# ska-telescope/ska-sdp-func-python

Measured on AMD Instinct MI355X. Metric: Mvis/s gridded (invert, 8k^2 w-stack grid) at 1/2/4/8 MI355X, higher is better.
Workload: dtype f32; 1 GPU; C2: SKA-MID 197 dishes, 64 chan x 100 times per GPU, 4096^2 image, 8192^2 w-stack grid; nvis_per_gpu=123558400, nchan_total=64, npix=4096, support=8, nplanes=9, parallelism=channel-sharded x1, 1 all-reduce

## Files before the change

### include/ska_sdp_hip.h

```cpp
#ifndef SKA_SDP_HIP_H
#define SKA_SDP_HIP_H

#include <stddef.h>
#include <stdint.h>

#ifdef __cplusplus
extern "C" {
#endif

#define SDP_HIP_OK 0
#define SDP_HIP_ERR_INVALID_ARG 1
#define SDP_HIP_ERR_RUNTIME 2
#define SDP_HIP_ERR_NO_DEVICE 3
#define SDP_HIP_ERR_MEMORY 4

#define SDP_HIP_F32 1
#define SDP_HIP_F64 2
#define SDP_HIP_C64 3
#define SDP_HIP_C128 4

#define SDP_HIP_FLIP_UW 1u
#define SDP_HIP_ACCUMULATE 2u
#define SDP_HIP_BATCH_FIRST 4u
#define SDP_HIP_BATCH_LAST 8u
#define SDP_HIP_KEEP_BUCKETS 16u
#define SDP_HIP_REUSE_BUCKETS 32u
#define SDP_HIP_FP32 64u
#define SDP_HIP_W_SLAB 128u
#define SDP_HIP_SLOT1 256u

typedef struct sdp_hip_wgrid_info {
    int support;
    double beta;
    int ngrid_x, ngrid_y;
    int nplanes;
    double w0, dw;
    int64_t nvis_used;
    int64_t nitems;
    int plane_chunk;
    float ms_prep, ms_grid, ms_fft, ms_screen;
    int bucket;
    int grid_launches;
    int padded;
    int fp64;
    int tiled;
    int folded;
    int layout_reused;
} sdp_hip_wgrid_info;

int sdp_hip_version(void);
int sdp_hip_device_count(int *count, char *errbuf, size_t errbuf_len);
int sdp_hip_release_workspace(char *errbuf, size_t errbuf_len);
int sdp_hip_set_stage_timing(int enable);

int sdp_hip_ms2dirty(const double *uvw, int64_t uvw_row_stride,
                     const double *freq, int nchan, int64_t nrow,
                     const void *vis, int vis_dtype, int64_t vis_row_stride,
                     int64_t vis_chan_stride, const void *wgt, int wgt_dtype,
                     int64_t wgt_row_stride, int64_t wgt_chan_stride,
                     int npix_x, int npix_y, double pixsize_x,
                     double pixsize_y, double epsilon, int do_wstacking,
                     unsigned flags, double *dirty, int64_t dirty_stride_x,
                     int64_t dirty_stride_y, void *stream,
                     sdp_hip_wgrid_info *info, char *errbuf,
                     size_t errbuf_len);

int sdp_hip_ms2dirty_batch(const double *uvw, int64_t uvw_row_stride,
                           const double *freq, int nchan, int64_t nrow,
                           const void *vis, int vis_dtype,
                           int64_t vis_row_stride, int64_t vis_chan_stride,
                           const void *wgt, int wgt_dtype, int64_t wgt_row_stride,
                           int64_t wgt_chan_stride, int npix_x, int npix_y,
                           double pixsize_x, double pixsize_y, double epsilon,
                           int do_wstacking, unsigned flags,
                           const double *bounds, double *dirty,
                           int64_t dirty_stride_x, int64_t dirty_stride_y,
                           void *stream, sdp_hip_wgrid_info *info,
                           char *errbuf, size_t errbuf_len);

int sdp_hip_wstack_layout(const double *bounds, int npix_x, int npix_y,
                          double pixsize_x, double pixsize_y, double epsilon,
                          int do_wstacking, unsigned flags, sdp_hip_wgrid_info *info,
                          char *errbuf, size_t errbuf_len);

int sdp_hip_wstack_fingerprint(const double *uvw, int64_t uvw_row_stride, int64_t nrow,
                               const double *freq, int nchan, uint64_t *out,
                               char *errbuf, size_t errbuf_len);

int sdp_hip_ms2dirty_vis(const double *uvw, int64_t uvw_row_stride,
                         const double *freq, int nchan, int64_t nrow,
                         const void *vis, int vis_dtype, int64_t vis_row_stride,
                         int64_t vis_chan_stride, int64_t vis_pol_stride,
                         int npol_vis, const double *pol_coeff, const void *wgt,
                         int wgt_dtype, int64_t wgt_row_stride,
                         int64_t wgt_chan_stride, const void *vis_flags,
                         int flag_bytes, int64_t flag_row_stride,
                         int64_t flag_chan_stride, int64_t flag_pol_stride,
                         int pol, int npix_x, int npix_y, double pixsize_x,
                         double pixsize_y, double epsilon, int do_wstacking,
                         unsigned flags, double *dirty, int64_t dirty_stride_x,
                         int64_t dirty_stride_y, double *sumwt,
                         const double *shift_lmn, void *stream,
                         sdp_hip_wgrid_info *info, char *errbuf,
                         size_t errbuf_len);

int sdp_hip_ms2dirty_vis_batch(const double *uvw, int64_t uvw_row_stride,
                               const double *freq, int nchan, int64_t nrow,
                               const void *vis, int vis_dtype, int64_t vis_row_stride,
                               int64_t vis_chan_stride, int64_t vis_pol_stride,
                               int npol_vis, const double *pol_coeff, const void *wgt,
                               int wgt_dtype, int64_t wgt_row_stride,
                               int64_t wgt_chan_stride, const void *vis_flags,
                               int flag_bytes, int64_t flag_row_stride,
                               int64_t flag_chan_stride, int64_t flag_pol_stride,
                               int pol, int npix_x, int npix_y, double pixsize_x,
                               double pixsize_y, double epsilon, int do_wstacking,
                               unsigned flags, const double *bounds, double *dirty,
                               int64_t dirty_stride_x, int64_t dirty_stride_y,
                               double *sumwt, const double *shift_lmn, void *stream,
                               sdp_hip_wgrid_info *info, char *errbuf,
                               size_t errbuf_len);

int sdp_hip_ms2dirty_vis_pols(const double *uvw, int64_t uvw_row_stride,
                              const double *freq, int nchan, int64_t nrow,
                              const void *vis, int vis_dtype, int64_t vis_row_stride,
                              int64_t vis_chan_stride, int64_t vis_pol_stride,
                              int npol_vis, const double *pol_coeff, int npol_img,
                              const void *wgt, int wgt_dtype, int64_t wgt_row_stride,
                              int64_t wgt_chan_stride, int64_t wgt_pol_stride,
                              const void *vis_flags, int flag_bytes,
// ... 294 lines not shown
```

### ska-sdp-func-python_amd/csrc/wstack.hip

```cpp
#include <hipcub/hipcub.hpp>
#include <hipfft/hipfft.h>

#include <algorithm>
#include <cmath>
#include <cstdio>
#include <cstdlib>
#include <functional>
#include <memory>
#include <mutex>
#include <tuple>
#include <type_traits>
#include <vector>

#include "sdp_common.h"
#include "wstack_fx_fft.h"
#include "wstack_types.h"
#include "wstack_bucket.h"

namespace sdp {
namespace wstack {

__global__ __launch_bounds__(64) void k_sum_slots(const double *__restrict__ slots, double *out) {
    double s = 0.0;
    for (int i = threadIdx.x; i < kSumSlots; i += 64) s += slots[i];
// ... 1065 lines not shown
                const float2 h = fbuf[fx_pad(X < 0 ? X + g.ngx : X)];
                if (g.do_w) {
                    const double l = X * g.px, r2 = l * l + m2;
                    const double sp = r2 < 1.0 ? r2 / (sqrt(1.0 - r2) + 1.0) - g.s0 : 0.0;
                    double ph = wq * sp;
                    ph -= rint(ph);
                    double sn, cs;
                    sincospi_t<float2>(2.0 * ph, &sn, &cs);
                    acc[m] += (double)h.x * cs - (double)h.y * sn;
                } else {
                    acc[m] += (double)h.x;
                }
            }
        }
        __syncthreads();
    }
#pragma unroll
    for (int m = 0; m < PX; ++m) {
        const int ix = t + m * S::T;
        if (ix < g.nx) {
            const PixelGeom p = pixel_geom(g, ix, iy, tab);
            const double res = p.inside ? acc[m] * p.corr : 0.0;
            double *o = dirty + ix * sx + iy * sy;
            *o = accumulate ? *o + res : res;
        }
    }
}

template <int LOGN>
__global__ __launch_bounds__(FxShape<LOGN>::T) __attribute__((amdgpu_waves_per_eu(4, 8))) void
k_screen_adj_xfft(Geo g, const double *__restrict__ dirty, int64_t sx, int64_t sy, int p_begin,
                  int np, float2 *__restrict__ spec, const double *__restrict__ tab,
                  const float2 *__restrict__ twg) {
    using S = FxShape<LOGN>;
    extern __shared__ float2 fbuf[];
    const int t = threadIdx.x, iy = blockIdx.x;
    float2 *const twl = fx_twl<LOGN>(fbuf, twg, t);
    float val[8];
#pragma unroll
    for (int e = 0; e < 8; ++e) {
        const int r = e < 4 ? e : e + 8;
        const int i = t + r * S::T;
        const int X = i < g.ngx / 2 ? i : i - g.ngx, ix = X + g.nx / 2;
        val[e] = 0.0f;
        if (ix >= 0 && ix < g.nx) {
            const PixelGeom p = pixel_geom(g, ix, iy, tab);
            val[e] = p.inside ? (float)(dirty[ix * sx + iy * sy] * p.corr) : 0.0f;
        }
    }
    const double mm = (iy - g.ny / 2) * g.py, m2 = mm * mm;
    const int64_t tplane = (int64_t)g.ny * g.ngx;
    const int pt = fx_pad(t);
    for (int q = 0; q < np; ++q) {
        const double wq = g.w0 + (p_begin + q) * g.dw;
        int tt = t;
        asm volatile("" : "+v"(tt));
        float2 v[16];
#pragma unroll
        for (int r = 0; r < 16; ++r) v[r] = make_float2(0.0f, 0.0f);
#pragma unroll
        for (int e = 0; e < 8; ++e) {
            const int r = e < 4 ? e : e + 8;
            const int i = tt + r * S::T;
            const int X = i < g.ngx / 2 ? i : i - g.ngx;
            if (val[e] != 0.0f) {
                if (g.do_w) {
                    const double l = X * g.px, r2 = l * l + m2;
                    const double sp = r2 / (sqrt(1.0 - r2) + 1.0) - g.s0;
                    double ph = wq * sp;
                    ph -= rint(ph);
                    double sn, cs;
                    sincospi_t<float2>(2.0 * ph, &sn, &cs);
                    v[r] = make_float2((float)(val[e] * cs), (float)(-val[e] * sn));
                } else {
                    v[r] = make_float2(val[e], 0.0f);
                }
            }
        }
        fx_fft<LOGN, -1>(v, fbuf, twl, t);
        float2 *o = spec + q * tplane + (int64_t)iy * g.ngx;
#pragma unroll
        for (int r = 0; r < 16; ++r) o[t + r * S::T] = fbuf[fx_padc<S::T>(t, pt, r * S::T)];
        __syncthreads();
    }
}

__device__ __forceinline__ void store_vis(float2 *p, float2 v, int accumulate) {
    if (accumulate) {
        const float2 o = *p;
        v.x += o.x;
        v.y += o.y;
    }
    *p = v;
}
__device__ __forceinline__ void store_vis(double2 *p, float2 v, int accumulate) {
    double2 w = make_double2(v.x, v.y);
    if (accumulate) {
        const double2 o = *p;
        w.x += o.x;
        w.y += o.y;
    }
    *p = w;
}
__device__ __forceinline__ void store_vis_d(float2 *p, double xr, double xi, int accumulate) {
    float2 w = make_float2((float)xr, (float)xi);
    if (accumulate) {
        const float2 o = *p;
        w.x += o.x;
        w.y += o.y;
    }
    *p = w;
}
__device__ __forceinline__ void store_vis_d(double2 *p, double xr, double xi, int accumulate) {
    double2 w = make_double2(xr, xi);
    if (accumulate) {
        const double2 o = *p;
        w.x += o.x;
        w.y += o.y;
    }
    *p = w;
}

struct OutConv {
    int npv = 1;
    int64_t vps = 0;
    double cre[4] = {1.0, 0.0, 0.0, 0.0}, cim[4] = {0.0, 0.0, 0.0, 0.0};
};

template <class VT>
__global__ void k_zero_vis(int64_t nrow, int nchan, VT *vis, int64_t vrs, int64_t vcs,
                           OutConv oc) {
    const int64_t v = blockIdx.x * (int64_t)blockDim.x + threadIdx.x;
    if (v >= nrow * nchan) return;
    const int64_t row = v / nchan;
    const int chan = (int)(v - row * nchan);
    VT z;
    z.x = 0;
    z.y = 0;
    for (int k = 0; k < oc.npv; ++k) vis[row * vrs + chan * vcs + k * oc.vps] = z;
}

template <class VT>
__global__ void k_finalize(int64_t n, int nchan,
                           const VisRec *__restrict__ recs, const float2 *__restrict__ acc, VT *vis,
                           int64_t vrs, int64_t vcs, int accumulate, OutConv oc) {
    for (int64_t r = blockIdx.x * (int64_t)blockDim.x + threadIdx.x; r < n;
         r += (int64_t)gridDim.x * blockDim.x) {
        const VisRec rc = recs[r];
        const float2 a = acc[r];
        const float2 v = make_float2(rc.cre * a.x - rc.cim * a.y, rc.cre * a.y + rc.cim * a.x);
        const int64_t row = rc.idx / (uint32_t)nchan;
        const int chan = (int)(rc.idx - row * nchan);
        VT *p = vis + row * vrs + chan * vcs;
        if (oc.npv == 1 && oc.cre[0] == 1.0 && oc.cim[0] == 0.0) {
            store_vis(p, v, accumulate);
            continue;
        }
        for (int k = 0; k < oc.npv; ++k) {
            if (oc.cre[k] == 0.0 && oc.cim[k] == 0.0) continue;
            const double xr = oc.cre[k] * v.x - oc.cim[k] * v.y;
            const double xi = oc.cre[k] * v.y + oc.cim[k] * v.x;
            store_vis_d(p + k * oc.vps, xr, xi, accumulate);
        }
    }
}

// ... 2632 lines not shown
    });
}

static void degrid_f64(const Plan &P, int p_lo, int p_hi, void *vis, int vis_dtype, int64_t vrs,
                int64_t vcs, int accumulate, const OutConv &oc, hipStream_t st) {
    SDP_REQUIRE(P.mfma64, "the fp64 predict needs one-cell buckets");
    dispatch_int<kMinW64, kMaxW64>(P.g.W, [&](auto w) {
        constexpr int W = decltype(w)::value;
        auto go = [&](auto *v) {
            using VT = std::remove_pointer_t<decltype(v)>;
            if (P.g.do_w)
                launch_degrid_f64_mfma<W, true, VT>(P, p_lo, p_hi, v, vrs, vcs, accumulate, oc, st);
            else
                launch_degrid_f64_mfma<W, false, VT>(P, p_lo, p_hi, v, vrs, vcs, accumulate, oc, st);
        };
        if (vis_dtype == SDP_HIP_C128) go(static_cast<double2 *>(vis));
        else go(static_cast<float2 *>(vis));
    });
}

static float2 *degrid_sink() {
    static float2 *sinks[64] = {};
    int dev = 0;
    SDP_HIP_CHECK(hipGetDevice(&dev));
    SDP_REQUIRE(dev >= 0 && dev < 64, "device index out of range");
    static std::mutex mu;
    std::lock_guard<std::mutex> lock(mu);
    if (!sinks[dev])
        SDP_HIP_CHECK(hipMalloc(&sinks[dev], (size_t)kDegridSinkBlocks * 64 * sizeof(float2)));
    return sinks[dev];
}

template <int W, bool WS>
static void launch_degrid_mfma(const Plan &P, int p_lo, int p_hi, float2 *acc, hipStream_t st) {
    const size_t lds = degrid_lds_bytes<W, WS>();
    const auto r = chunk_items(P, p_lo, p_hi);
    const unsigned per = P.subsort ? 16u : 1u;
    const unsigned n = per * (r.second - r.first);
    if (n == 0) return;
    float2 *const sink = degrid_sink();
    if (P.vdirect)
        k_degrid_mfma<W, WS, true><<<n, 64, lds, st>>>(
            P.g, P.recs, n, P.pt.fitems + per * (size_t)r.first, P.grid, p_lo, p_hi, P.vdirect, sink);
    else
        k_degrid_mfma<W, WS, false><<<n, 64, lds, st>>>(
            P.g, P.recs, n, P.pt.fitems + per * (size_t)r.first, P.grid, p_lo, p_hi, acc, sink);
}

static void grid_f32(const Plan &P, int p_lo, int p_hi, hipStream_t st) {
    dispatch_int<2, kMaxW>(P.g.W, [&](auto w) {
        constexpr int W = decltype(w)::value;
        if (P.g.do_w) launch_grid_mfma_pad<W, true>(P, p_lo, p_hi, st);
        else launch_grid_mfma_pad<W, false>(P, p_lo, p_hi, st);
    });
}

static void degrid_f32(const Plan &P, int p_lo, int p_hi, float2 *acc, hipStream_t st) {
    dispatch_int<2, kMaxW>(P.g.W, [&](auto w) {
        constexpr int W = decltype(w)::value;
        if (P.g.do_w) launch_degrid_mfma<W, true>(P, p_lo, p_hi, acc, st);
        else launch_degrid_mfma<W, false>(P, p_lo, p_hi, acc, st);
    });
}

static void fill_info(const Plan &P, sdp_hip_wgrid_info *info) {
    if (!info) return;
    info->support = P.g.W;
    info->beta = P.g.beta;
    info->ngrid_x = P.g.ngx;
    info->ngrid_y = P.g.ngy;
    info->nplanes = P.g.nplanes;
    info->w0 = P.g.w0;
    info->dw = P.g.dw;
    info->nvis_used = P.pt.nrec;
    info->nitems = P.pt.nitems;
    info->plane_chunk = P.chunk_planes;
    info->bucket = P.g.sub;
    info->padded = (P.pad4 || P.subpad || P.pad64) ? 1 : 0;
    info->fp64 = P.f64 ? 1 : 0;
    info->tiled = P.g.tiled;
    info->grid_launches = (P.g.nplanes + P.chunk_planes - 1) / P.chunk_planes;
    info->folded = P.g.fold;
    info->layout_reused = 0;
}

static void exec_fft(hipfftHandle h, bool f64, void *in, void *out, int direction) {
    const hipfftResult r =
        f64 ? hipfftExecZ2Z(h, (hipfftDoubleComplex *)in, (hipfftDoubleComplex *)out, direction)
            : hipfftExecC2C(h, (hipfftComplex *)in, (hipfftComplex *)out, direction);
    if (r != HIPFFT_SUCCESS) throw Error(SDP_HIP_ERR_RUNTIME, "hipfftExec failed");
}

static void *plane_ptr(const Plan &P, int q, size_t e) {
    return reinterpret_cast<char *>(P.grid) +
           ((size_t)q * P.g.ngx * P.g.ngy + e) * cbytes(P);
}

static void fft_rows_y(const Plan &P, int q0, int np, int direction, hipStream_t st) {
    const Geo &g = P.g;
    const int nrow = P.row_hi - P.row_lo;
    if (nrow <= 0) return;
    hipfftHandle hr = fft_plan_1d(g.ngy, 1, g.ngy, nrow, st, P.f64);
    for (int q = q0; q < q0 + np; ++q) {
        void *p = plane_ptr(P, q, (size_t)P.row_lo * g.ngy);
        exec_fft(hr, P.f64, p, p, direction);
    }
}

static void fft_rows_x(const Plan &P, int np, int direction, hipStream_t st,
                       void *in = nullptr) {
    const Geo &g = P.g;
    hipfftHandle hc = fft_plan_1d(g.ngx, 1, g.ngx, np * g.ny, st, P.f64);
    exec_fft(hc, P.f64, in ? in : (void *)P.spec, P.spec, direction);
}

static void zero_band(const Plan &P, int np, hipStream_t st) {
    const Geo &g = P.g;
    if (P.row_hi <= P.row_lo || np <= 0) return;
    const size_t width = (size_t)(P.row_hi - P.row_lo) * g.ngy * cbytes(P);
    for (int q = 0; q < np; ++q)
        SDP_HIP_CHECK(hipMemsetAsync(plane_ptr(P, q, (size_t)P.row_lo * g.ngy), 0, width, st));
    if (P.core.p)
        SDP_HIP_CHECK(hipMemsetAsync(P.core.p, 0,
                                     (size_t)np * P.core.nx * P.core.ny * sizeof(double2), st));
}

static void setup_core(Plan &P) {
    P.core = CoreAcc{nullptr, 0, 0, 0, 0};
    const int cw = env_int("SDP_HIP_CORE", 128);
    if (P.f64 || cw <= 0) return;
    const Geo &g = P.g;
    const int x0 = std::max(P.row_lo, g.ngx / 2 - cw / 2), x1 = std::min(P.row_hi, g.ngx / 2 + cw / 2);
    const int y0 = std::max(0, g.ngy / 2 - cw / 2), y1 = std::min(g.ngy, g.ngy / 2 + cw / 2);
    if (x1 <= x0 || y1 <= y0) return;
    P.core = CoreAcc{scratch<double>("core64", (size_t)P.chunk_planes * (x1 - x0) * (y1 - y0) * 2),
                     x0, x1 - x0, y0, y1 - y0};
}

__global__ __launch_bounds__(256) void k_core_merge(float2 *__restrict__ grid, int ngx, int ngy,
                                                    CoreAcc c, int q0, int np) {
    const int64_t per = (int64_t)c.nx * c.ny, n = per * np;
    for (int64_t i = blockIdx.x * (int64_t)blockDim.x + threadIdx.x; i < n;
         i += (int64_t)gridDim.x * blockDim.x) {
        const int q = (int)(i / per);
        const int64_t e = i - q * per;
        const int x = (int)(e / c.ny), y = (int)(e - (int64_t)x * c.ny);
        const double2 v = reinterpret_cast<const double2 *>(c.p)[(int64_t)(q0 + q) * per + e];
        float2 &o = grid[((int64_t)(q0 + q) * ngx + c.x0 + x) * ngy + c.y0 + y];
        o = make_float2((float)((double)o.x + v.x), (float)((double)o.y + v.y));
    }
}

static void core_merge(const Plan &P, int q0, int np, hipStream_t st) {
    if (!P.core.p || np <= 0) return;
    const int64_t n = (int64_t)P.core.nx * P.core.ny * np;
    k_core_merge<<<(unsigned)std::min<int64_t>((n + 255) / 256, 8192), 256, 0, st>>>(
        P.grid, P.g.ngx, P.g.ngy, P.core, q0, np);
    SDP_HIP_CHECK(hipGetLastError());
}

static dim3 tr_grid(const Geo &g, int xrows, int np) {
    return dim3((unsigned)((xrows + kTr - 1) / kTr), (unsigned)((g.ny + kTr - 1) / kTr),
                (unsigned)np);
}

static bool tr16(const Geo &g) {
// ... 30 lines not shown
        k_tr_t_to_grid<double2><<<grd, blk, 0, st>>>(
            g, reinterpret_cast<const double2 *>(P.spec),
            static_cast<double2 *>(plane_ptr(P, q0, 0)), P.row_lo, P.row_hi);
    else if (tr16(g))
        k_tr_t_to_grid16<<<tr_grid16(g, P.row_lo, P.row_hi, nb), blk, 0, st>>>(
            g, P.spec, static_cast<float2 *>(plane_ptr(P, q0, 0)), P.row_lo, P.row_hi);
    else
        k_tr_t_to_grid<float2><<<grd, blk, 0, st>>>(
            g, P.spec, static_cast<float2 *>(plane_ptr(P, q0, 0)), P.row_lo, P.row_hi);
    SDP_HIP_CHECK(hipGetLastError());
}

static void screen_fwd(const Plan &P, int p_begin, int nb, double *dirty, int64_t sx, int64_t sy,
                       int accumulate, const double *tab, hipStream_t st) {
    const Geo &g = P.g;
    const dim3 grd(grid1d(g.nx, 256), g.ny);
    if (P.f64)
        k_screen_fwd_t<double2><<<grd, 256, 0, st>>>(g, reinterpret_cast<const double2 *>(P.spec),
                                                     p_begin, nb, dirty, sx, sy, accumulate, tab);
    else
        k_screen_fwd_t<float2><<<grd, 256, 0, st>>>(g, P.spec, p_begin, nb, dirty, sx, sy,
                                                    accumulate, tab);
    SDP_HIP_CHECK(hipGetLastError());
}

static void screen_adj(const Plan &P, const double *dirty, int64_t sx, int64_t sy, int p_begin,
                       int nb, const double *tab, hipStream_t st) {
    const Geo &g = P.g;
    const dim3 grd(grid1d(g.nx, 256), g.ny);
    if (P.f64)
        k_screen_adj_t<double2><<<grd, 256, 0, st>>>(g, dirty, sx, sy, p_begin, nb,
                                                     reinterpret_cast<double2 *>(P.spec_adj), tab);
    else
        k_screen_adj_t<float2><<<grd, 256, 0, st>>>(g, dirty, sx, sy, p_begin, nb, P.spec_adj, tab);
    SDP_HIP_CHECK(hipGetLastError());
}

static int xfft_log2(const Plan &P) {
    const int on = env_int("SDP_HIP_XFFT_FUSED", 1);
    const int n = P.g.ngx;
    if (P.f64 || !on || n <= 0 || (n & (n - 1)) || 2 * P.g.nx > n) return 0;
    int l = 0;
    while ((1 << l) < n) ++l;
    return (l >= 7 && l <= 14) ? l : 0;
}

template <int LOGN>
static const float2 *fx_twiddles(hipStream_t st) {
    using S = FxShape<LOGN>;
    static const std::vector<float2> host = [] {
        std::vector<float2> h(S::TW);
        auto root = [](long num, long den) {
            const long double a = 2.0L * 3.14159265358979323846264338327950288L * num / den;
            return make_float2((float)std::cos(a), (float)std::sin(a));
        };
        for (int p = 1, ns = 16; p < S::P16; ++p, ns *= 16)
            for (int k = 0; k < ns; ++k) {
                h[S::tw_off(p) + 2 * k] = root(k, 16L * ns);
                h[S::tw_off(p) + 2 * k + 1] = root(4L * k, 16L * ns);
            }
        for (int t = 0; t < S::T; ++t) h[S::tw_off(S::P16) + t] = root(t, S::N);
        return h;
    }();
    float2 *d = scratch<float2>("fx_tw_" + std::to_string(LOGN), S::TW);
    SDP_HIP_CHECK(hipMemcpyAsync(d, host.data(), S::TW * sizeof(float2), hipMemcpyHostToDevice, st));
    return d;
}

template <int LOGN>
static void launch_xfft_screen_fwd(const Plan &P, int p_begin, int nb, double *dirty, int64_t sx,
                                   int64_t sy, int accumulate, const double *tab, hipStream_t st) {
    using S = FxShape<LOGN>;
    constexpr size_t lds = S::lds_bytes();
    static const bool attr = [] {
        SDP_HIP_CHECK(hipFuncSetAttribute((const void *)k_xfft_screen_fwd<LOGN>,
                                          hipFuncAttributeMaxDynamicSharedMemorySize, (int)lds));
        return true;
    }();
    (void)attr;
    k_xfft_screen_fwd<LOGN><<<P.g.ny, S::T, lds, st>>>(P.g, P.spec_in, P.row_lo, P.row_hi, p_begin,
                                                       nb, dirty, sx, sy, accumulate, tab,
                                                       fx_twiddles<LOGN>(st));
    SDP_HIP_CHECK(hipGetLastError());
}

static void xfft_screen_fwd(const Plan &P, int p_begin, int nb, double *dirty, int64_t sx,
                            int64_t sy, int accumulate, const double *tab, hipStream_t st,
                            StageTimer &t2) {
    if (const int l = xfft_log2(P)) {
        t2.mark();
        dispatch_int<7, 14>(l, [&](auto L) {
            launch_xfft_screen_fwd<decltype(L)::value>(P, p_begin, nb, dirty, sx, sy, accumulate,
                                                       tab, st);
        });
    } else {
        fft_rows_x(P, nb, HIPFFT_BACKWARD, st, P.spec_in);
        t2.mark();
        screen_fwd(P, p_begin, nb, dirty, sx, sy, accumulate, tab, st);
    }
    t2.mark();
}

template <int LOGN>
static void launch_screen_adj_xfft(const Plan &P, const double *dirty, int64_t sx, int64_t sy,
                                   int p_begin, int nb, const double *tab, hipStream_t st) {
    using S = FxShape<LOGN>;
    constexpr size_t lds = S::lds_bytes();
    static const bool attr = [] {
        SDP_HIP_CHECK(hipFuncSetAttribute((const void *)k_screen_adj_xfft<LOGN>,
                                          hipFuncAttributeMaxDynamicSharedMemorySize, (int)lds));
        return true;
    }();
    (void)attr;
    k_screen_adj_xfft<LOGN><<<P.g.ny, S::T, lds, st>>>(P.g, dirty, sx, sy, p_begin, nb, P.spec,
                                                       tab, fx_twiddles<LOGN>(st));
    SDP_HIP_CHECK(hipGetLastError());
}

static void screen_adj_xfft(const Plan &P, const double *dirty, int64_t sx, int64_t sy,
                            int p_begin, int nb, const double *tab, hipStream_t st,
                            StageTimer &t2) {
    if (const int l = xfft_log2(P)) {
        dispatch_int<7, 14>(l, [&](auto L) {
            launch_screen_adj_xfft<decltype(L)::value>(P, dirty, sx, sy, p_begin, nb, tab, st);
        });
        t2.mark();
    } else {
        screen_adj(P, dirty, sx, sy, p_begin, nb, tab, st);
        t2.mark();
        fft_rows_x(P, nb, HIPFFT_FORWARD, st, P.spec_adj);
    }
}

static int cu_count() {
    static std::mutex mu;
    static std::map<int, int> cus;
    int dev = 0;
    SDP_HIP_CHECK(hipGetDevice(&dev));
    std::lock_guard<std::mutex> lk(mu);
    auto it = cus.find(dev);
    if (it != cus.end()) return it->second;
    int n = 0;
    SDP_HIP_CHECK(hipDeviceGetAttribute(&n, hipDeviceAttributeMultiprocessorCount, dev));
    cus[dev] = std::max(n, 1);
    return cus[dev];
}

static void bucket_tiled(Plan &P, const Inputs &in, bool grid_mode, hipStream_t st,
                         bool values_only, const std::function<void()> &after_clear,
                         double *slots, bool record = false, bool replay = false) {
    const Geo &g = P.g;
    Part &pt = P.pt;
    const int nb = g.nbins;
    const int kind = P.f64 ? 3 : (grid_mode ? 0 : 1);
    const size_t rsz = kind == 3 ? sizeof(Rec64) : kind == 0 ? sizeof(RecC) : sizeof(VisRec);
    const int64_t nvis = pt.nvis;
    const size_t lds_bins = (size_t)nb * sizeof(unsigned);
    if (!values_only) {
        pt.t_g1 = env_int("SDP_HIP_TG1", 16) * cu_count();
        while (pt.t_g1 > cu_count() && (int64_t)pt.t_g1 * nb > nvis / 2) pt.t_g1 /= 2;
        pt.t_vpw = std::max<int64_t>(kT1Threads, (nvis + pt.t_g1 - 1) / pt.t_g1);
        pt.t_vpw = (pt.t_vpw + 63) / 64 * 64;
        pt.t_g1 = (int)std::max<int64_t>(1, (nvis + pt.t_vpw - 1) / pt.t_vpw);
        pt.t_maxch = (unsigned)(nvis / kTChunk + nb + 1);
        pt.t_maxseg = (unsigned)(nvis / ((int64_t)kTChunk * kTSeg) + nb + 1);
        pt.t_binc = scratch<unsigned>("t_binc", nb);
// ... 290 lines not shown
    explicit SlotGuard(unsigned flags) {
        const bool one = flags & SDP_HIP_SLOT1;
        SDP_REQUIRE(!one || !(flags & (SDP_HIP_KEEP_BUCKETS | SDP_HIP_REUSE_BUCKETS |
                                       SDP_HIP_BATCH_FIRST | SDP_HIP_BATCH_LAST |
                                       SDP_HIP_W_SLAB)),
                    "SDP_HIP_SLOT1 cannot be combined with kept / reused buckets, batches or "
                    "w slabs");
        ws_slot() = one ? 1 : 0;
    }
    ~SlotGuard() { ws_slot() = 0; }
};

struct AuxWork {
    hipStream_t st;
    hipEvent_t done = nullptr;
    explicit AuxWork(hipStream_t s) : st(s) {}
    AuxWork(const AuxWork &) = delete;
    AuxWork &operator=(const AuxWork &) = delete;
    template <class F>
    void start(F work) {
        hipStream_t aux = aux_stream();
        stream_after(aux, st);
        work(aux);
        SDP_HIP_CHECK(hipEventCreateWithFlags(&done, hipEventDisableTiming));
        SDP_HIP_CHECK(hipEventRecord(done, aux));
    }
    bool join() {
        if (!done) return false;
        SDP_HIP_CHECK(hipStreamWaitEvent(st, done, 0));
        hipEvent_t e = done;
        done = nullptr;
        SDP_HIP_CHECK(hipEventDestroy(e));
        return true;
    }
    ~AuxWork() {
        if (!done) return;
        (void)hipStreamWaitEvent(st, done, 0);
        (void)hipEventDestroy(done);
    }
};

struct StageMs {
    float grid = 0, fft = 0, screen = 0;
};

static void finish_info(const Plan &P, StageTimer &tm, const StageMs &ms,
                        sdp_hip_wgrid_info *info) {
    tm.mark();
    fill_info(P, info);
    if (!info) return;
    info->ms_prep = tm.on ? tm.ms(0, 1) - ms.grid - ms.fft - ms.screen : 0.0f;
    info->ms_grid = ms.grid;
    info->ms_fft = ms.fft;
    info->ms_screen = ms.screen;
}

static void zero_first_band(AuxWork &aux, const Plan &P) {
    if (env_int("SDP_HIP_ZERO_OVERLAP", 1) == 0) return;
    aux.start([&](hipStream_t s) { zero_band(P, std::min(P.g.nplanes, P.chunk_planes), s); });
}

static void invert_planes(const Plan &P, double *dirty, int64_t sx, int64_t sy, int accumulate,
                          bool first, bool last, const double *tab, AuxWork &aux, StageMs &ms,
                          hipStream_t st) {
    const Geo &g = P.g;
    for (int p_lo = 0; p_lo < g.nplanes; p_lo += P.chunk_planes) {
        const int p_hi = std::min(g.nplanes, p_lo + P.chunk_planes);
        const int np = p_hi - p_lo;
        if (!aux.join() && first) zero_band(P, np, st);
        {
            StageTimer tg(st);
            tg.mark();
            if (P.f64) grid_f64(P, p_lo, p_hi, st);
            else grid_f32(P, p_lo, p_hi, st);
            SDP_HIP_CHECK(hipGetLastError());
            tg.mark();
            ms.grid += tg.ms(0, 1);
        }
        if (last) core_merge(P, 0, np, st);
        for (int sb = 0; last && sb < np; sb += P.fft_planes) {
            const int nb = std::min(P.fft_planes, np - sb);
            StageTimer t2(st);
            t2.mark();
            fft_rows_y(P, sb, nb, HIPFFT_BACKWARD, st);
            tr_grid_to_t(P, sb, nb, st);
            xfft_screen_fwd(P, p_lo + sb, nb, dirty, sx, sy, (accumulate || p_lo + sb > 0) ? 1 : 0,
                            tab, st, t2);
            ms.fft += t2.ms(0, 1);
            ms.screen += t2.ms(1, 2);
        }
    }
    aux.join();
}

static void ms2dirty(const Inputs &in, double *dirty, int64_t sx, int64_t sy,
                     sdp_hip_wgrid_info *info, hipStream_t st) {
    SDP_REQUIRE(in.vis == nullptr || in.vis_dtype == SDP_HIP_C64 ||
                    in.vis_dtype == SDP_HIP_C128,
                "vis must be complex64 or complex128");
    SlotGuard slot(in.flags);
    StageTimer tm(st);
    tm.mark();
    const bool keep = in.flags & SDP_HIP_KEEP_BUCKETS, reuse = in.flags & SDP_HIP_REUSE_BUCKETS;
    SDP_REQUIRE(!(keep && reuse), "SDP_HIP_KEEP_BUCKETS and SDP_HIP_REUSE_BUCKETS exclude each other");
    SDP_REQUIRE(in.bounds == nullptr || !(keep || reuse),
                "batched inverts do not keep or reuse bucketings");
    Inputs inx = in;
    inx.x.all = keep || reuse;
    const bool cacheable = !keep && !reuse && !in.bounds && !(in.flags & SDP_HIP_W_SLAB) &&
                           !(in.eps < 1.0e-7 && !(in.flags & SDP_HIP_FP32)) && in.nrow > 0 &&
                           env_int("SDP_HIP_LAYOUT_CACHE", 1) != 0;
    BoundsOut bo;
    LayoutKey lkey;
    bool hit = false;
    Plan P;
    if (cacheable) {
        bo = bounds_pass(in, st);
        lkey = layout_key(in, bo);
        hit = find_kept_layout(lkey, P);
    }
    if (hit) {
        if (ws_slot() == 0) {
            drop_kept_buckets();
            drop_batch_seq();
        }
        inx.x.all = true;
    } else {
        P = reuse ? reuse_buckets(in) : plan_geometry(inx, true, st, cacheable ? &bo : nullptr);
    }
    setup_core(P);
    const Geo &g = P.g;
    const bool batched = in.bounds != nullptr;
    const bool first = !batched || (in.flags & SDP_HIP_BATCH_FIRST);
    const bool last = !batched || (in.flags & SDP_HIP_BATCH_LAST);
    if (batched) {
        SDP_REQUIRE(P.chunk_planes == g.nplanes,
                    "batched invert: the w planes do not all fit in device memory");
        check_batch_seq(P, in, first);
    }
    const double *tab = phi_table(g.W, g.beta, st);
    AuxWork aux(st);
    auto start_zero = [&] {
        if (first && !batched) zero_first_band(aux, P);
    };
    if (reuse || hit) {
        start_zero();
        double *slots = in.x.sumwt ? scratch<double>("sumwt_slots", kSumSlots) : nullptr;
        if (slots) SDP_HIP_CHECK(hipMemsetAsync(slots, 0, kSumSlots * sizeof(double), st));
        const bool replay = hit && P.pt.t_pos != nullptr;
        if (P.g.tiled) bucket_tiled(P, inx, true, st, true, nullptr, slots, hit && !replay, replay);
        else bucket_part(P, inx, true, st, true);
        if (slots) sum_slots(slots, in.x.sumwt, st);
        if (hit && !replay && P.pt.t_pos) keep_layout(lkey, P);
    } else {
        bucket_all(P, inx, true, st, start_zero,
                   cacheable && env_int("SDP_HIP_LAYOUT_RECORD", 0) == 1);
    }
    if (P.subsort) subsort_items(P, st);
    if (keep) keep_buckets(P, in);
    if (cacheable && !hit && P.g.tiled && !P.f64 && P.pad4 && !P.pt.dropped) keep_layout(lkey, P);
    StageMs ms;
    invert_planes(P, dirty, sx, sy, (in.flags & SDP_HIP_ACCUMULATE) ? 1 : 0, first, last, tab, aux,
                  ms, st);
    if (batched && last) drop_batch_seq();
    finish_info(P, tm, ms, info);
    if (info) info->layout_reused = hit ? 1 : 0;
}

static void set_pol_row(VisExtra &x, const PolsSpec &ps, int q) {
    x.conv = true;
    for (int k = 0; k < 4; ++k) {
        x.cre[k] = ps.cre[q][k];
        x.cim[k] = ps.cim[q][k];
    }
    x.fpol = q;
}

static void ms2dirty_pols(const Inputs &in, PolsSpec ps, double *const *dirty, int64_t sx,
                          int64_t sy, double *const *sumwt, sdp_hip_wgrid_info *info,
                          hipStream_t st) {
    SDP_REQUIRE(ps.npo >= 1 && ps.npo <= 4, "npol_img must be 1..4");
    SDP_REQUIRE(in.vis != nullptr && (in.vis_dtype == SDP_HIP_C64 || in.vis_dtype == SDP_HIP_C128),
                "vis must be complex64 or complex128");
    SDP_REQUIRE(ps.npo <= in.x.npv, "npol_img must not exceed npol_vis (pol q's flags mask its "
                                    "weights)");
    auto per_pol = [&](bool share) {
        for (int q = 0; q < ps.npo; ++q) {
            Inputs iq = in;
            set_pol_row(iq.x, ps, q);
            iq.wgt = static_cast<const char *>(ps.wgt) +
                     q * ps.wps * (in.x.wgt_f64 ? sizeof(double) : sizeof(float));
            iq.x.sumwt = sumwt[q];
            iq.flags = in.flags & ~(SDP_HIP_KEEP_BUCKETS | SDP_HIP_REUSE_BUCKETS);
            if (share && ps.npo > 1)
                iq.flags |= q == 0 ? SDP_HIP_KEEP_BUCKETS : SDP_HIP_REUSE_BUCKETS;
            ms2dirty(iq, dirty[q], sx, sy, q == ps.npo - 1 ? info : nullptr, st);
        }
    };
    if (in.eps < 1.0e-7 && !(in.flags & SDP_HIP_FP32)) return per_pol(false);
    SlotGuard slot(in.flags);
    StageTimer tm(st);
    tm.mark();
    Inputs inx = in;
    set_pol_row(inx.x, ps, 0);
    inx.x.all = true;
    inx.x.sumwt = nullptr;
    inx.flags = (in.flags & ~SDP_HIP_REUSE_BUCKETS) | SDP_HIP_KEEP_BUCKETS;
    Plan P = plan_geometry(inx, true, st);
    if (P.f64 || P.g.tiled || P.g.sub != kTileCell || !P.pad4 || P.subpad) return per_pol(true);
    setup_core(P);
    const double *tab = phi_table(P.g.W, P.g.beta, st);
    AuxWork aux(st);
    double *slots = scratch<double>("sumwt_slots_pols", 4 * kSumSlots);
    SDP_HIP_CHECK(hipMemsetAsync(slots, 0, 4 * kSumSlots * sizeof(double), st));
    for (int q = 0; q < ps.npo; ++q) ps.slots[q] = sumwt[q] ? slots + q * kSumSlots : nullptr;
    bucket_part(P, inx, true, st, false, [&] { zero_first_band(aux, P); }, &ps);
    for (int q = 0; q < ps.npo; ++q)
        if (sumwt[q]) sum_slots(ps.slots[q], sumwt[q], st);
    read_part_meta(P, st);
    StageMs ms;
    for (int q = 0; q < ps.npo; ++q) {
        P.recs = reinterpret_cast<VisRec *>(ps.recs[q]);
        invert_planes(P, dirty[q], sx, sy, (in.flags & SDP_HIP_ACCUMULATE) ? 1 : 0, true, true, tab,
                      aux, ms, st);
    }
    finish_info(P, tm, ms, info);
}

static void dirty2ms(const Inputs &in, int npo, const double *const *img, const OutConv *oc,
                     int64_t sx, int64_t sy, void *vis, sdp_hip_wgrid_info *info,
                     hipStream_t st) {
    SDP_REQUIRE(in.vis_dtype == SDP_HIP_C64 || in.vis_dtype == SDP_HIP_C128,
                "vis must be complex64 or complex128");
    SlotGuard slot(in.flags);
    StageTimer tm(st);
    tm.mark();
    Plan P = plan_geometry(in, false, st);
    const Geo &g = P.g;
    const double *tab = phi_table(g.W, g.beta, st);
    const int accumulate = (in.flags & SDP_HIP_ACCUMULATE) ? 1 : 0;
    const int64_t nvis = in.nrow * (int64_t)in.nchan;
    const bool trivial_oc = oc[0].npv == 1 && oc[0].cre[0] == 1.0 && oc[0].cim[0] == 0.0;
    if (npo == 1 && P.chunk_planes == g.nplanes && !accumulate && in.vis_dtype != SDP_HIP_C128 &&
        trivial_oc && in.vcs == 1 && in.vrs == in.nchan && !P.f64) {
        P.vdirect = static_cast<float2 *>(vis);
        if (!g.tiled) P.zout = P.vdirect;
    }
    auto zero_vis_unless_fused = [&](hipStream_t s) {
        if (!P.zout && !accumulate) zero_vis(in, vis, oc[0], s);
    };
    std::vector<std::unique_ptr<StageTimer>> stage_t;
    auto plane_stage = [&](int p_lo, int np, hipStream_t s, const double *image) {
        for (int sb = 0; sb < np; sb += P.fft_planes) {
            const int nb = std::min(P.fft_planes, np - sb);
            stage_t.emplace_back(new StageTimer(s));
            StageTimer &t2 = *stage_t.back();
            t2.mark();
            screen_adj_xfft(P, image, sx, sy, p_lo + sb, nb, tab, s, t2);
            tr_t_to_grid(P, sb, nb, s);
            fft_rows_y(P, sb, nb, HIPFFT_FORWARD, s);
            t2.mark();
        }
    };
    const bool overlap = env_int("SDP_HIP_ZERO_OVERLAP", 1) != 0;
    const bool planes_aux = overlap && P.chunk_planes == g.nplanes;
    AuxWork aux(st);
    auto start_aux = [&] {
        if (!overlap) return;
        aux.start([&](hipStream_t s) {
            zero_vis_unless_fused(s);
            zero_band(P, std::min(g.nplanes, P.chunk_planes), s);
            if (planes_aux) plane_stage(0, g.nplanes, s, img[0]);
        });
    };
    if (!overlap) zero_vis_unless_fused(st);
    bucket_all(P, in, false, st, start_aux);
    if (P.subsort) subsort_items(P, st);
    float2 *accs[4] = {};
    if (!(P.vdirect || P.f64)) {
        static const char *names[4] = {"degrid_acc", "degrid_acc1", "degrid_acc2", "degrid_acc3"};
        for (int q = 0; q < npo; ++q) {
            accs[q] = scratch<float2>(names[q], std::max<int64_t>(nvis, 1));
            SDP_HIP_CHECK(
                hipMemsetAsync(accs[q], 0, std::max<int64_t>(nvis, 1) * sizeof(float2), st));
        }
    }
    StageMs ms;
    for (int q = 0; q < npo; ++q)
        for (int p_lo = 0; p_lo < g.nplanes; p_lo += P.chunk_planes) {
            const int p_hi = std::min(g.nplanes, p_lo + P.chunk_planes);
            const int np = p_hi - p_lo;
            if (aux.join()) {
                if (!planes_aux) plane_stage(p_lo, np, st, img[q]);
            } else {
                zero_band(P, np, st);
                plane_stage(p_lo, np, st, img[q]);
            }
            StageTimer tg(st);
            tg.mark();
            if (P.f64) degrid_f64(P, p_lo, p_hi, vis, in.vis_dtype, in.vrs, in.vcs, 1, oc[q], st);
            else degrid_f32(P, p_lo, p_hi, accs[q], st);
            SDP_HIP_CHECK(hipGetLastError());
            tg.mark();
            ms.grid += tg.ms(0, 1);
        }
    aux.join();
    for (auto &t : stage_t) {
        ms.screen += t->ms(0, 1);
        ms.fft += t->ms(1, 2);
// ... 405 lines not shown
```

### ska-sdp-func-python_amd/csrc/wstack_fx_fft.h

```cpp
#pragma once

#include <hip/hip_runtime.h>

namespace sdp {
namespace wstack {

__device__ __forceinline__ float2 cmulf(float2 a, float2 b) {
    return make_float2(a.x * b.x - a.y * b.y, a.x * b.y + a.y * b.x);
}

template <int SG>
__device__ __forceinline__ float2 root16(int m) {
    constexpr float c16[16] = {1.0f,
                               0.92387953251128673848f,
                               0.70710678118654752440f,
                               0.38268343236508978178f,
                               0.0f,
                               -0.38268343236508978178f,
                               -0.70710678118654752440f,
                               -0.92387953251128673848f,
                               -1.0f,
                               -0.92387953251128673848f,
                               -0.70710678118654752440f,
                               -0.38268343236508978178f,
                               0.0f,
                               0.38268343236508978178f,
                               0.70710678118654752440f,
                               0.92387953251128673848f};
    m &= 15;
    return make_float2(c16[m], SG * c16[(m + 12) & 15]);
}

template <int R, int SG>
__device__ __forceinline__ void fx_dft(float2 *v) {
#pragma unroll
    for (int L = R; L >= 2; L >>= 1) {
        const int h = L >> 1;
#pragma unroll
        for (int s = 0; s < R; s += L) {
#pragma unroll
            for (int k = 0; k < h; ++k) {
                const float2 a = v[s + k], b = v[s + k + h];
                v[s + k] = make_float2(a.x + b.x, a.y + b.y);
                const float2 d = make_float2(a.x - b.x, a.y - b.y);
                v[s + k + h] = k == 0 ? d : cmulf(d, root16<SG>(k * (16 / L)));
            }
        }
    }
}

template <int R>
__device__ __forceinline__ constexpr int fx_brev(int r) {
    int o = 0;
    for (int b = 1, t = R >> 1; b < R; b <<= 1, t >>= 1)
        if (r & b) o |= t;
    return o;
}

__device__ __forceinline__ int fx_pad(int i) { return i + (i >> 4); }
template <int T>
__device__ __forceinline__ int fx_padc(int t, int pt, int c) {
    if constexpr (T % 16 == 0) return pt + (c / 16) * 17;
    else return fx_pad(t + c);
}

__device__ __forceinline__ void fx_powers(const float2 (&b)[4], float2 *w) {
    w[1] = b[0];
    w[2] = b[1];
    w[3] = cmulf(b[1], b[0]);
    w[4] = b[2];
    w[5] = cmulf(b[2], b[0]);
    w[6] = cmulf(b[2], b[1]);
    w[7] = cmulf(b[2], w[3]);
#pragma unroll
    for (int r = 1; r < 8; ++r) w[8 + r] = cmulf(b[3], w[r]);
    w[8] = b[3];
}

template <int LOGN>
struct FxShape {
    static constexpr int N = 1 << LOGN;
    static constexpr int T = N / 16;
    static constexpr int P16 = LOGN / 4;
    static constexpr int RR = 1 << (LOGN % 4);
    static constexpr int LDS = N + N / 16;
    static constexpr int tw_off(int p) { return p <= 1 ? 0 : tw_off(p - 1) + 2 * (1 << (4 * (p - 1))); }
    static constexpr int TW = tw_off(P16) + T;
    static constexpr size_t lds_bytes() { return (size_t)(LDS + TW) * 8; }
};

template <int LOGN, int SG>
__device__ __forceinline__ void fx_fft(float2 (&v)[16], float2 *buf, const float2 *__restrict__ twt,
                                       int t) {
    using S = FxShape<LOGN>;
    fx_dft<16, SG>(v);
    {
        float2 *const o = buf + 17 * t;
#pragma unroll
        for (int r = 0; r < 16; ++r) o[r] = v[fx_brev<16>(r)];
    }
    __syncthreads();
    const int pt = fx_pad(t);
    int ns = 16;
#pragma unroll
    for (int p = 1; p < S::P16; ++p) {
#pragma unroll
        for (int r = 0; r < 16; ++r) v[r] = buf[fx_padc<S::T>(t, pt, r * S::T)];
        __syncthreads();
        const int k = t % ns, d = (t / ns) * ns * 16 + k;
        {
            int kk = k;
            asm volatile("" : "+v"(kk));
            float2 b[4], w[16];
            const float4 q0 = *reinterpret_cast<const float4 *>(twt + S::tw_off(p) + 2 * kk);
            b[0] = make_float2(q0.x, SG * q0.y);
            b[2] = make_float2(q0.z, SG * q0.w);
            b[1] = cmulf(b[0], b[0]);
            b[3] = cmulf(b[2], b[2]);
            fx_powers(b, w);
#pragma unroll
            for (int r = 1; r < 16; ++r) v[r] = cmulf(v[r], w[r]);
        }
        fx_dft<16, SG>(v);
        const int pd = fx_pad(d);
#pragma unroll
        for (int r = 0; r < 16; ++r) buf[pd + r * ns + ((r * ns) >> 4)] = v[fx_brev<16>(r)];
        __syncthreads();
        ns *= 16;
    }
    if constexpr (S::RR > 1) {
        constexpr int RR = S::RR, NB = 16 / RR, STR = S::N / RR;
        int tt = t;
        asm volatile("" : "+v"(tt));
        const float2 l0 = twt[S::tw_off(S::P16) + tt], last = make_float2(l0.x, SG * l0.y);
#pragma unroll
        for (int m = 0; m < NB; ++m) {
            float2 u[RR];
            [[maybe_unused]] const int j = t + S::T * m;
#pragma unroll
            for (int r = 0; r < RR; ++r) u[r] = buf[fx_padc<S::T>(t, pt, S::T * m + r * STR)];
            const float2 wj = m == 0 ? last : cmulf(last, root16<SG>(m));
            float2 wr = wj;
#pragma unroll
            for (int r = 1; r < RR; ++r) {
                u[r] = cmulf(u[r], wr);
                if (r + 1 < RR) wr = cmulf(wr, wj);
            }
            fx_dft<RR, SG>(u);
#pragma unroll
            for (int r = 0; r < RR; ++r) buf[fx_padc<S::T>(t, pt, S::T * m + r * STR)] = u[fx_brev<RR>(r)];
        }
        __syncthreads();
    }
}

template <int LOGN>
__device__ __forceinline__ float2 *fx_twl(float2 *fbuf, const float2 *__restrict__ twg, int t) {
    using S = FxShape<LOGN>;
    float2 *const twl = fbuf + S::LDS;
    for (int i = t; i < S::TW; i += S::T) twl[i] = twg[i];
    __syncthreads();
    return twl;
}

}
}
```

### ska-sdp-func-python_amd/ska_sdp_func_python_amd/_lib.py

```python

import ctypes
import os
import threading

_HERE = os.path.dirname(os.path.abspath(__file__))
LIB_PATH = os.environ.get("SDP_HIP_LIB_OVERRIDE") or os.path.join(_HERE, "_lib", "libska_sdp_hip.so")

SDP_HIP_OK = 0
SDP_HIP_ERR_INVALID_ARG = 1
SDP_HIP_ERR_RUNTIME = 2
SDP_HIP_ERR_NO_DEVICE = 3
SDP_HIP_ERR_MEMORY = 4

SDP_HIP_F32 = 1
SDP_HIP_F64 = 2
SDP_HIP_C64 = 3
SDP_HIP_C128 = 4

SDP_HIP_FLIP_UW = 1
SDP_HIP_ACCUMULATE = 2
SDP_HIP_BATCH_FIRST = 4
SDP_HIP_BATCH_LAST = 8
SDP_HIP_KEEP_BUCKETS = 16
SDP_HIP_REUSE_BUCKETS = 32
SDP_HIP_FP32 = 64
SDP_HIP_W_SLAB = 128
SDP_HIP_SLOT1 = 256

SDP_HIP_CLEAN_HOGBOM = 0
SDP_HIP_CLEAN_MSCLEAN = 1
SDP_HIP_MFSCLEAN_FINDPEAK_RASCIL = 0
SDP_HIP_MFSCLEAN_FINDPEAK_CASA = 1
SDP_HIP_STOKES_IQUV = 0
SDP_HIP_STOKES_I = 1
SDP_HIP_SKYCOMP_TILE_X = 32
SDP_HIP_SKYCOMP_TILE_Y = 8
SDP_HIP_MIX_PLANES_REGS = 8
SDP_HIP_MIX_PLANES_MAX = 4096
SDP_HIP_MIX_NAN_INPUT = 1
SDP_HIP_MIX_NAN_OUTPUT = 2
SDP_HIP_GATHER_FACETS_MAX = 256
SDP_HIP_SEGMENT_TILE = 32
SDP_HIP_SEGMENT_KERNEL_MAX = 15
SDP_HIP_GAIN_CHAIN_MAX = 8
SDP_HIP_GAUSS_FIT_WINDOW = 15
SDP_HIP_BANDPASS_MAX_DEGREE = 7
SDP_HIP_BANDPASS_MAX_SEGMENTS = 64

c_i64 = ctypes.c_int64
c_int = ctypes.c_int
c_dbl = ctypes.c_double
c_vp = ctypes.c_void_p
c_u32 = ctypes.c_uint
c_size = ctypes.c_size_t
c_char_p = ctypes.c_char_p


class WGridInfo(ctypes.Structure):
    _fields_ = [
        ("support", c_int),
        ("beta", c_dbl),
        ("ngrid_x", c_int),
        ("ngrid_y", c_int),
        ("nplanes", c_int),
        ("w0", c_dbl),
        ("dw", c_dbl),
        ("nvis_used", c_i64),
        ("nitems", c_i64),
        ("plane_chunk", c_int),
        ("ms_prep", ctypes.c_float),
        ("ms_grid", ctypes.c_float),
        ("ms_fft", ctypes.c_float),
        ("ms_screen", ctypes.c_float),
        ("bucket", c_int),
        ("grid_launches", c_int),
        ("padded", c_int),
        ("fp64", c_int),
        ("tiled", c_int),
        ("folded", c_int),
        ("layout_reused", c_int),
    ]

    def as_dict(self):
        return {name: getattr(self, name) for name, _ in self._fields_}


_ERR = [c_char_p, c_size]
SIGNATURES = {
    "sdp_hip_version": [],
    "sdp_hip_device_count": [ctypes.POINTER(c_int)] + _ERR,
    "sdp_hip_release_workspace": _ERR,
    "sdp_hip_set_stage_timing": [c_int],
    "sdp_hip_ms2dirty": [
        c_vp, c_i64, c_vp, c_int, c_i64,
        c_vp, c_int, c_i64, c_i64,
        c_vp, c_int, c_i64, c_i64,
        c_int, c_int, c_dbl, c_dbl, c_dbl, c_int, c_u32,
        c_vp, c_i64, c_i64,
        c_vp, ctypes.POINTER(WGridInfo)] + _ERR,
    "sdp_hip_ms2dirty_batch": [
        c_vp, c_i64, c_vp, c_int, c_i64,
        c_vp, c_int, c_i64, c_i64,
        c_vp, c_int, c_i64, c_i64,
        c_int, c_int, c_dbl, c_dbl, c_dbl, c_int, c_u32,
        c_vp,
        c_vp, c_i64, c_i64,
        c_vp, ctypes.POINTER(WGridInfo)] + _ERR,
    "sdp_hip_wstack_layout": [
        c_vp, c_int, c_int, c_dbl, c_dbl, c_dbl, c_int, c_u32,
        ctypes.POINTER(WGridInfo)] + _ERR,
    "sdp_hip_wstack_fingerprint": [c_vp, c_i64, c_i64, c_vp, c_int, c_vp] + _ERR,
    "sdp_hip_ms2dirty_vis": [
        c_vp, c_i64, c_vp, c_int, c_i64,
        c_vp, c_int, c_i64, c_i64, c_i64, c_int,
        c_vp,
        c_vp, c_int, c_i64, c_i64,
        c_vp, c_int, c_i64, c_i64, c_i64, c_int,
        c_int, c_int, c_dbl, c_dbl, c_dbl, c_int, c_u32,
        c_vp, c_i64, c_i64, c_vp,
        c_vp,
        c_vp, ctypes.POINTER(WGridInfo)] + _ERR,
    "sdp_hip_ms2dirty_vis_pols": [
        c_vp, c_i64, c_vp, c_int, c_i64,
        c_vp, c_int, c_i64, c_i64, c_i64, c_int,
        c_vp, c_int,
        c_vp, c_int, c_i64, c_i64, c_i64,
        c_vp, c_int, c_i64, c_i64, c_i64,
        c_int, c_int, c_dbl, c_dbl, c_dbl, c_int, c_u32,
        c_vp, c_i64, c_i64, c_i64,
        c_vp, c_i64,
        c_vp,
        c_vp, ctypes.POINTER(WGridInfo)] + _ERR,
    "sdp_hip_ms2dirty_vis_batch": [
        c_vp, c_i64, c_vp, c_int, c_i64,
        c_vp, c_int, c_i64, c_i64, c_i64, c_int,
        c_vp,
        c_vp, c_int, c_i64, c_i64,
        c_vp, c_int, c_i64, c_i64, c_i64, c_int,
        c_int, c_int, c_dbl, c_dbl, c_dbl, c_int, c_u32,
        c_vp,
        c_vp, c_i64, c_i64, c_vp,
        c_vp,
        c_vp, ctypes.POINTER(WGridInfo)] + _ERR,
    "sdp_hip_dirty2ms": [
        c_vp, c_i64, c_vp, c_int, c_i64,
        c_vp, c_i64, c_i64, c_int, c_int, c_dbl, c_dbl,
        c_vp, c_int, c_i64, c_i64,
        c_dbl, c_int, c_u32,
        c_vp, c_int, c_i64, c_i64,
        c_vp, ctypes.POINTER(WGridInfo)] + _ERR,
    "sdp_hip_dirty2ms_vis": [
        c_vp, c_i64, c_vp, c_int, c_i64,
        c_vp, c_i64, c_i64, c_int, c_int, c_dbl, c_dbl,
        c_dbl, c_int, c_u32,
        c_vp, c_int, c_i64, c_i64, c_i64, c_int,
        c_vp,
        c_vp,
        c_vp, ctypes.POINTER(WGridInfo)] + _ERR,
    "sdp_hip_dirty2ms_vis_pols": [
        c_vp, c_i64, c_vp, c_int, c_i64,
        c_vp, c_i64, c_i64, c_i64, c_int,
        c_int, c_int, c_dbl, c_dbl,
        c_dbl, c_int, c_u32,
# ... 171 lines not shown
```

Before: 17210 Mvis/s.

## Fuse y-direction FFT with crop and transpose into one LDS kernel

Replaces the hipFFT column FFT followed by a separate grid-to-transposed copy with a custom kernel. Each block loads a group of grid rows, runs the in-LDS radix-16 FFT, crops to the image rows and writes the transposed output with vectorised 16-byte stores. The aim is to drop one full read and write of every w-plane and the hipFFT launch overhead in the invert path. A leaner twiddle-power variant of the shared FFT routine cuts register pressure. The kernel keeps several rows of output in registers, which may limit occupancy.

```diff
diff --git a/include/ska_sdp_hip.h b/include/ska_sdp_hip.h
--- a/include/ska_sdp_hip.h
+++ b/include/ska_sdp_hip.h
@@ -46,6 +46,8 @@
     int tiled;
     int folded;
     int layout_reused;
+    int yfft_fused;
+    int band_row_lo, band_row_hi;
 } sdp_hip_wgrid_info;
 
 int sdp_hip_version(void);
diff --git a/ska-sdp-func-python_amd/csrc/wstack.hip b/ska-sdp-func-python_amd/csrc/wstack.hip
--- a/ska-sdp-func-python_amd/csrc/wstack.hip
+++ b/ska-sdp-func-python_amd/csrc/wstack.hip
@@ -1171,6 +1171,72 @@
 #pragma unroll
         for (int r = 0; r < 16; ++r) o[t + r * S::T] = fbuf[fx_padc<S::T>(t, pt, r * S::T)];
         __syncthreads();
+    }
+}
+
+constexpr int kYR = 8;
+template <int LOGN, int R>
+__global__ __launch_bounds__(FxShape<LOGN>::T) __attribute__((amdgpu_waves_per_eu(R == 8 ? 2 : 4)))
+void k_yfft_crop_t(
+    Geo g, const float2 *__restrict__ grid, float2 *__restrict__ tout, int row_lo, int row_hi,
+    const float2 *__restrict__ twg) {
+    using S = FxShape<LOGN>;
+    constexpr int KO = 8;
+    constexpr int LPG = 16 / R;
+    static_assert(R % 2 == 0 && 16 % R == 0, "row groups tile a 128-byte line in 16-byte stores");
+    extern __shared__ float2 fbuf[];
+    const int t = threadIdx.x, q = blockIdx.y;
+    const int w = blockIdx.x % (8 * LPG);
+    const int gi = ((blockIdx.x / (8 * LPG)) * 8 + (w & 7)) * LPG + (w >> 3);
+    const int x0 = (row_lo & ~15) + gi * R;
+    if (x0 >= row_hi || x0 + R <= row_lo) return;
+    float2 *const twl = fx_twl<LOGN>(fbuf, twg, t);
+    const float2 *const src = grid + (int64_t)q * g.ngx * g.ngy;
+    auto valid = [&](int j) { return x0 + j >= row_lo && x0 + j < row_hi; };
+    auto load = [&](float2(&v)[16], int j) {
+        const int x = min(max(x0 + j, row_lo), row_hi - 1);
+        const float2 *const rowp = src + (int64_t)x * g.ngy;
+#pragma unroll
+        for (int r = 0; r < 16; ++r) v[r] = rowp[(unsigned)(t + r * S::T)];
+    };
+    constexpr bool EARLY = R == 8;
+    float2 out[R][KO];
+    float2 vv[EARLY ? 2 : 1][16];
+    load(vv[0], 0);
+#pragma unroll
+    for (int j = 0; j < R; ++j) {
+        float2(&v)[16] = vv[EARLY ? j & 1 : 0];
+        float2(&vn)[16] = vv[EARLY ? (j + 1) & 1 : 0];
+        if (EARLY && j + 1 < R) load(vn, j + 1);
+        fx_fft<LOGN, 1, !EARLY>(v, fbuf, twl, t);
+        if (!EARLY && j + 1 < R) load(vn, j + 1);
+        int tt = t;
+        asm volatile("" : "+v"(tt));
+#pragma unroll
+        for (int m = 0; m < KO; ++m) {
+            const int iy = tt + m * S::T;
+            const int Y = iy - g.ny / 2;
+            out[j][m] = iy < g.ny ? fbuf[fx_pad(Y < 0 ? Y + g.ngy : Y)] : make_float2(0.0f, 0.0f);
+        }
+        __syncthreads();
+    }
+    const bool full = x0 >= row_lo && x0 + R <= row_hi;
+    float2 *const dst = tout + (int64_t)q * g.ny * g.ngx + x0;
+#pragma unroll
+    for (int m = 0; m < KO; ++m) {
+        const int iy = t + m * S::T;
+        if (iy >= g.ny) continue;
+        float2 *const o = dst + (int64_t)iy * g.ngx;
+        if (full) {
+#pragma unroll
+            for (int j = 0; j < R; j += 2)
+                *reinterpret_cast<float4 *>(o + j) =
+                    make_float4(out[j][m].x, out[j][m].y, out[j + 1][m].x, out[j + 1][m].y);
+        } else {
+#pragma unroll
+            for (int j = 0; j < R; ++j)
+                if (valid(j)) o[j] = out[j][m];
+        }
     }
 }
 
@@ -3969,6 +4035,9 @@
     info->grid_launches = (P.g.nplanes + P.chunk_planes - 1) / P.chunk_planes;
     info->folded = P.g.fold;
     info->layout_reused = 0;
+    info->yfft_fused = 0;
+    info->band_row_lo = P.row_lo;
+    info->band_row_hi = P.row_hi;
 }
 
 static void exec_fft(hipfftHandle h, bool f64, void *in, void *out, int direction) {
@@ -4165,6 +4234,46 @@
                                                        nb, dirty, sx, sy, accumulate, tab,
                                                        fx_twiddles<LOGN>(st));
     SDP_HIP_CHECK(hipGetLastError());
+}
+
+static int yfft_log2(const Plan &P) {
+    const int n = P.g.ngy;
+    if (P.f64 || !xfft_log2(P) || env_int("SDP_HIP_YFFT_FUSED", 1) == 0) return 0;
+    if (n <= 0 || (n & (n - 1)) || 2 * P.g.ny > n) return 0;
+    int l = 0;
+    while ((1 << l) < n) ++l;
+    return (l >= 7 && l <= 14) ? l : 0;
+}
+
+template <int LOGN, int R>
+static void launch_yfft_crop_t(const Plan &P, int q0, int nb, hipStream_t st) {
+    using S = FxShape<LOGN>;
+    constexpr size_t lds = S::lds_bytes();
+    static const bool attr = [] {
+        SDP_HIP_CHECK(hipFuncSetAttribute((const void *)k_yfft_crop_t<LOGN, R>,
+                                          hipFuncAttributeMaxDynamicSharedMemorySize, (int)lds));
+        return true;
+    }();
+    (void)attr;
+    const int lines = (P.row_hi - (P.row_lo & ~15) + 15) / 16;
+    const dim3 grd((unsigned)((lines + 7) / 8 * 8 * (16 / R)), (unsigned)nb);
+    k_yfft_crop_t<LOGN, R><<<grd, S::T, lds, st>>>(
+        P.g, static_cast<const float2 *>(plane_ptr(P, q0, 0)), P.spec_in, P.row_lo, P.row_hi,
+        fx_twiddles<LOGN>(st));
+    SDP_HIP_CHECK(hipGetLastError());
+}
+
+static void yfft_to_t(const Plan &P, int q0, int nb, hipStream_t st) {
+    if (P.row_hi <= P.row_lo) return;
+    if (const int l = yfft_log2(P)) {
+        dispatch_int<7, 14>(l, [&](auto L) {
+            constexpr int LG = decltype(L)::value;
+            launch_yfft_crop_t<LG, LG == 14 ? 2 : kYR>(P, q0, nb, st);
+        });
+    } else {
+        fft_rows_y(P, q0, nb, HIPFFT_BACKWARD, st);
+        tr_grid_to_t(P, q0, nb, st);
+    }
 }
 
 static void xfft_screen_fwd(const Plan &P, int p_begin, int nb, double *dirty, int64_t sx,
@@ -4621,8 +4730,7 @@
             const int nb = std::min(P.fft_planes, np - sb);
             StageTimer t2(st);
             t2.mark();
-            fft_rows_y(P, sb, nb, HIPFFT_BACKWARD, st);
-            tr_grid_to_t(P, sb, nb, st);
+            yfft_to_t(P, sb, nb, st);
             xfft_screen_fwd(P, p_lo + sb, nb, dirty, sx, sy, (accumulate || p_lo + sb > 0) ? 1 : 0,
                             tab, st, t2);
             ms.fft += t2.ms(0, 1);
@@ -4703,7 +4811,10 @@
                   ms, st);
     if (batched && last) drop_batch_seq();
     finish_info(P, tm, ms, info);
-    if (info) info->layout_reused = hit ? 1 : 0;
+    if (info) {
+        info->layout_reused = hit ? 1 : 0;
+        info->yfft_fused = (last && yfft_log2(P)) ? 1 : 0;
+    }
 }
 
 static void set_pol_row(VisExtra &x, const PolsSpec &ps, int q) {
@@ -4764,6 +4875,7 @@
                       aux, ms, st);
     }
     finish_info(P, tm, ms, info);
+    if (info) info->yfft_fused = yfft_log2(P) ? 1 : 0;
 }
 
 static void dirty2ms(const Inputs &in, int npo, const double *const *img, const OutConv *oc,
diff --git a/ska-sdp-func-python_amd/csrc/wstack_fx_fft.h b/ska-sdp-func-python_amd/csrc/wstack_fx_fft.h
--- a/ska-sdp-func-python_amd/csrc/wstack_fx_fft.h
+++ b/ska-sdp-func-python_amd/csrc/wstack_fx_fft.h
@@ -89,7 +89,7 @@
     static constexpr size_t lds_bytes() { return (size_t)(LDS + TW) * 8; }
 };
 
-template <int LOGN, int SG>
+template <int LOGN, int SG, bool LEAN = false>
 __device__ __forceinline__ void fx_fft(float2 (&v)[16], float2 *buf, const float2 *__restrict__ twt,
                                        int t) {
     using S = FxShape<LOGN>;
@@ -117,9 +117,25 @@
             b[2] = make_float2(q0.z, SG * q0.w);
             b[1] = cmulf(b[0], b[0]);
             b[3] = cmulf(b[2], b[2]);
-            fx_powers(b, w);
+            if constexpr (LEAN) {
+                w[1] = b[0];
+                w[2] = b[1];
+                w[3] = cmulf(b[1], b[0]);
+                w[4] = b[2];
+                w[5] = cmulf(b[2], b[0]);
+                w[6] = cmulf(b[2], b[1]);
+                w[7] = cmulf(b[2], w[3]);
+                v[8] = cmulf(v[8], b[3]);
 #pragma unroll
-            for (int r = 1; r < 16; ++r) v[r] = cmulf(v[r], w[r]);
+                for (int r = 1; r < 8; ++r) {
+                    v[8 + r] = cmulf(v[8 + r], cmulf(b[3], w[r]));
+                    v[r] = cmulf(v[r], w[r]);
+                }
+            } else {
+                fx_powers(b, w);
+#pragma unroll
+                for (int r = 1; r < 16; ++r) v[r] = cmulf(v[r], w[r]);
+            }
         }
         fx_dft<16, SG>(v);
         const int pd = fx_pad(d);
diff --git a/ska-sdp-func-python_amd/ska_sdp_func_python_amd/_lib.py b/ska-sdp-func-python_amd/ska_sdp_func_python_amd/_lib.py
--- a/ska-sdp-func-python_amd/ska_sdp_func_python_amd/_lib.py
+++ b/ska-sdp-func-python_amd/ska_sdp_func_python_amd/_lib.py
@@ -79,6 +79,9 @@
         ("tiled", c_int),
         ("folded", c_int),
         ("layout_reused", c_int),
+        ("yfft_fused", c_int),
+        ("band_row_lo", c_int),
+        ("band_row_hi", c_int),
     ]
 
     def as_dict(self):
```

Measured after the change: 17360 Mvis/s, median of 6. Within noise of the previous version (+0.8%).
